# unixpickle/vq-voice-swap

Measured on AMD Instinct MI355X. Metric: audio clips/sec (whole node), unet64 50-step DDPM on 4s@16kHz waveforms, higher is better.
Workload: dtype fp16; 1 GPU; unet64 50-step DDPM (constrain, schedule t**2), 64 clips/GPU x 1 GPU of T=64000; global_batch=64, parallelism=clips sharded over 1 GPU(s), gather to rank 0

## Files before the change

### vq_voice_swap_amd/csrc/common.hpp

```cpp
#pragma once

#include <hip/hip_runtime.h>
#include <stdint.h>

#include <cstdio>
#include <string>

namespace vqvs {

void set_error(const std::string& msg);
#define VQVS_FAIL(code, ...)                        \
  do {                                              \
    char _buf[512];                                 \
    snprintf(_buf, sizeof(_buf), __VA_ARGS__);      \
    ::vqvs::set_error(_buf);                        \
    return (code);                                  \
  } while (0)
#define VQVS_HIP(expr)                                                                       \
  do {                                                                                       \
    hipError_t _e = (expr);                                                                  \
    if (_e != hipSuccess) VQVS_FAIL(-2, "%s failed: %s (%s:%d)", #expr, hipGetErrorString(_e), __FILE__, __LINE__); \
  } while (0)

typedef __bf16 bf16_t;
// ... 55 lines not shown
    f32x2 p = fma2(splat2(0.0000430638f), z, splat2(0.0002765672f));
    p = fma2(p, z, splat2(0.0001520143f));
    p = fma2(p, z, splat2(0.0092705272f));
    p = fma2(p, z, splat2(0.0422820123f));
    p = fma2(p, z, splat2(0.0705230784f));
    p = fma2(p, z, splat2(1.0f));
    p = p * p;
    p = p * p;
    p = p * p;
    p = p * p;
    f32x2 e;
    e[0] = copysignf(1.0f - __builtin_amdgcn_rcpf(p[0]), v[0]);
    e[1] = copysignf(1.0f - __builtin_amdgcn_rcpf(p[1]), v[1]);
    return (v * splat2(0.5f)) * (e + splat2(1.0f));
  } else {
    f32x2 vc;
    vc[0] = __builtin_amdgcn_fmed3f(v[0], -4.0f, 4.0f);
    vc[1] = __builtin_amdgcn_fmed3f(v[1], -4.0f, 4.0f);
    const f32x2 w = vc * vc;
    f32x2 p;
    if constexpr (Q == GELU_POLY6) {
      p = fma2(splat2(2.81608722e-08f), w, splat2(-1.89188380e-06f));
      p = fma2(p, w, splat2(5.41903041e-05f));
      p = fma2(p, w, splat2(-8.78980255e-04f));
      p = fma2(p, w, splat2(9.11294959e-03f));
      p = fma2(p, w, splat2(-6.53883549e-02f));
      p = fma2(p, w, splat2(3.98526915e-01f));
    } else {
      p = fma2(splat2(-1.301278171e-09f), w, splat2(1.041951057e-07f));
      p = fma2(p, w, splat2(-3.657111166e-06f));
      p = fma2(p, w, splat2(7.485478930e-05f));
      p = fma2(p, w, splat2(-1.006488756e-03f));
      p = fma2(p, w, splat2(9.505392772e-03f));
      p = fma2(p, w, splat2(-6.588783436e-02f));
      p = fma2(p, w, splat2(3.986733897e-01f));
    }
    return v * fma2(vc, p, splat2(0.5f));
  }
}
template <typename T> struct GeluQ;
template <> struct GeluQ<float> { static constexpr int q = GELU_EXACT; };
template <> struct GeluQ<bf16_t> { static constexpr int q = GELU_POLY6; };
#ifdef VQVS_F16_GELU6
template <> struct GeluQ<half_t> { static constexpr int q = GELU_POLY6; };
#else
template <> struct GeluQ<half_t> { static constexpr int q = GELU_POLY7; };
#endif

template <typename T>
struct Elem;
template <>
struct Elem<float> {
  static constexpr int BYTES = 4;
  __device__ static __forceinline__ f32x8 load8(const float* p) {
    const f32x4 a = *reinterpret_cast<const f32x4*>(p);
    const f32x4 b = *reinterpret_cast<const f32x4*>(p + 4);
    return f32x8{a[0], a[1], a[2], a[3], b[0], b[1], b[2], b[3]};
  }
  __device__ static __forceinline__ void store8(float* p, f32x8 v) {
    *reinterpret_cast<f32x4*>(p) = f32x4{v[0], v[1], v[2], v[3]};
    *reinterpret_cast<f32x4*>(p + 4) = f32x4{v[4], v[5], v[6], v[7]};
  }
};
template <>
struct Elem<bf16_t> {
  static constexpr int BYTES = 2;
  __device__ static __forceinline__ f32x8 load8(const bf16_t* p) {
    const bf16x8 a = *reinterpret_cast<const bf16x8*>(p);
    return __builtin_convertvector(a, f32x8);
  }
  __device__ static __forceinline__ void store8(bf16_t* p, f32x8 v) {
    *reinterpret_cast<bf16x8*>(p) = __builtin_convertvector(v, bf16x8);
  }
};

template <>
struct Elem<half_t> {
  static constexpr int BYTES = 2;
  __device__ static __forceinline__ f32x8 load8(const half_t* p) {
    const f16x8 a = *reinterpret_cast<const f16x8*>(p);
    return __builtin_convertvector(a, f32x8);
  }
  __device__ static __forceinline__ void store8(half_t* p, f32x8 v) {
    *reinterpret_cast<f16x8*>(p) = __builtin_convertvector(v, f16x8);
  }
};

#define VQVS_BY_PRECISION(precision, CALL) \
  do {                                      \
    if ((precision) == 0) {                 \
      using T = float;                      \
      CALL;                                 \
    } else if ((precision) == 1) {          \
      using T = ::vqvs::bf16_t;             \
      CALL;                                 \
    } else {                                \
      using T = ::vqvs::half_t;             \
      CALL;                                 \
    }                                       \
  } while (0)

__device__ __forceinline__ f32x8 f32x8_zero() { return f32x8{0, 0, 0, 0, 0, 0, 0, 0}; }

__device__ __forceinline__ void split_bf16(f32x8 v, bf16x8& hi, bf16x8& lo) {
  hi = __builtin_convertvector(v, bf16x8);
  const f32x8 r = v - __builtin_convertvector(hi, f32x8);
  lo = __builtin_convertvector(r, bf16x8);
}

}
```

### vq_voice_swap_amd/csrc/kernels.hpp

```cpp
#pragma once

#include "common.hpp"

namespace vqvs {

enum { RESIZE_NONE = 0, RESIZE_AVG2 = 1, RESIZE_UP2 = 2 };

struct SegDesc {
  const void* src;
  const float2* ss;
  long long w_off;
  int Csrc;
  int c0;
  int C;
  int Lsrc;
  int ntaps;
  int dil;
  int resize;
  int ss_stride, ss_c0;
  const void* src2;
  const float4* coef;
  int coef_stride, coef_c0;
};

// ... 48 lines not shown
};
int launch_in_conv(const InConvArgs& a, int B, int precision, hipStream_t st);

struct OutConvArgs {
  const void* in;
  const float2* ss;
  const float* w;
  float bias;
  float* out;
  int C, L;
};
int launch_out_conv(const OutConvArgs& a, int B, int precision, hipStream_t st);

struct GnSrc {
  const float* partials;
  int ntiles, C;
};
struct GnArgs {
  GnSrc src[2];
  int nsrc, Ctot, groups;
  double inv_count;
  const float* gamma;
  const float* beta;
  const float* film;
  int film_stride, film_off;
  float2* ss;
  float2* mr;
  unsigned* status;
  int guard;
};
int launch_gn_prepare(const GnArgs& a, int B, hipStream_t st);

struct TimeEmbedArgs {
  const float* ts;
  const float* freqs;
  const float *w1, *b1;
  const float *w2, *b2;
  const float* class_embed;
  const int64_t* labels;
  int num_labels;
  float* emb;
  float* gemb;
  int E;
};
int launch_time_embed(const TimeEmbedArgs& a, int B, hipStream_t st);
int launch_gelu_rows(const float* in, float* out, int n, hipStream_t st);

struct FilmArgs {
  const float* gemb;
  const float* w;
  const float* bias;
  float* film;
  int E, R;
};
int launch_film(const FilmArgs& a, int B, hipStream_t st);

struct XformArgs {
  const void* in;
  const float2* ss;
  void* out;
  int C, Lin, Lout, avg, ss_stride, ss_c0;
};
int launch_xform(const XformArgs& a, int B, int precision, hipStream_t st);

enum { BW_SAME = 0, BW_FROM_HALF = 1, BW_FROM_DOUBLE = 2 };
struct BwActArgs {
  const void* t;
  const void* xf;
  const float2* ss;
  void* du;
  float* partials;
  int C, L, resize;
  int t_C, t_c0, du_C, du_c0, ss_stride, ss_c0, part_C, part_c0;
};
int launch_bw_act(const BwActArgs& a, int B, int precision, hipStream_t st);

struct GnBwArgs {
  const float* partials;
  int ntiles, C, groups;
  double inv_count;
  const float2* ss;
  const float2* mr;
  float4* coef;
};
int launch_gn_bw(const GnBwArgs& a, int B, hipStream_t st);

struct BwAffineArgs {
  const void* du;
  const void* xf;
  const float4* coef;
  const void* skip;
  int skip_mode;
  const void* extra;
  void* out;
  int C, L;
  int du_C, du_c0, coef_stride, coef_c0, extra_C, extra_c0;
};
int launch_bw_affine(const BwAffineArgs& a, int B, int precision, hipStream_t st);
int launch_bw_add(const void* a, const void* b, void* out, long long n, int precision, hipStream_t st);

struct InConvBwArgs {
  const void* dh;
  const float* w;
  float* out;
  int C, T;
  float out_scale;
// ... 70 lines not shown
```

### vq_voice_swap_amd/csrc/misc_kernels.hip

```cpp
#include <atomic>

#include "kernels.hpp"

namespace vqvs {

namespace {

template <typename T, bool MC>
__global__ __launch_bounds__(256) void in_conv_kernel(const InConvArgs a) {
  __shared__ float red[256 * 8 * 2];
  const int tid = threadIdx.x;
  const int b = blockIdx.y;
  const int t0 = blockIdx.x * STAT_TILE;
  const int opr = a.C >> 3;
  const int rpp = 256 / opr;
  const int oct = tid % opr;
  const int r0 = tid / opr;
  const int c = oct * 8;
  float w0[8], w1[8], w2[8], bs[8];
  const int Cin = MC ? a.Cin : 1;
#pragma unroll
  for (int j = 0; j < 8; ++j) {
    w0[j] = a.w[(c + j) * Cin * 3 + 0];
    w1[j] = a.w[(c + j) * Cin * 3 + 1];
    w2[j] = a.w[(c + j) * Cin * 3 + 2];
    bs[j] = a.bias[c + j];
  }
  const float* xb = a.x + (size_t)b * Cin * a.T;
  f32x8 s1 = f32x8_zero(), s2 = f32x8_zero();
  const bool active = r0 < rpp && oct < opr;
  const float cond_scale = a.condp ? (float)a.cond_len / (float)a.T : 0.f;
  if (active) {
    for (int r = r0; r < STAT_TILE; r += rpp) {
      const int t = t0 + r;
      if (t >= a.T) break;
      const float xm = t > 0 ? xb[t - 1] : 0.f;
      const float x0 = xb[t];
      const float xp = t + 1 < a.T ? xb[t + 1] : 0.f;
      f32x8 v;
#pragma unroll
      for (int j = 0; j < 8; ++j) v[j] = fmaf(w2[j], xp, fmaf(w1[j], x0, fmaf(w0[j], xm, bs[j])));
      if constexpr (MC)
      for (int ci = 1; ci < Cin; ++ci) {
        const float* xc = xb + (size_t)ci * a.T;
        const float ym = t > 0 ? xc[t - 1] : 0.f, y0 = xc[t], yp = t + 1 < a.T ? xc[t + 1] : 0.f;
#pragma unroll
        for (int j = 0; j < 8; ++j) {
          const float* wc = a.w + ((c + j) * Cin + ci) * 3;
          v[j] = fmaf(wc[2], yp, fmaf(wc[1], y0, fmaf(wc[0], ym, v[j])));
        }
      }
      if (a.condp) {
        const int cr = min((int)floorf((float)t * cond_scale), a.cond_len - 1);
        const T* cp = reinterpret_cast<const T*>(a.condp) + ((size_t)b * a.cond_len + cr) * a.C + c;
        v += Elem<T>::load8(cp);
      }
      s1 += v;
      s2 += v * v;
      Elem<T>::store8(reinterpret_cast<T*>(a.out) + ((size_t)b * a.T + t) * a.C + c, v);
    }
  }
  if (active) {
#pragma unroll
    for (int j = 0; j < 8; ++j) {
      red[(r0 * a.C + c + j) * 2 + 0] = s1[j];
      red[(r0 * a.C + c + j) * 2 + 1] = s2[j];
    }
  }
  __syncthreads();
  if (tid < a.C) {
    float t1 = 0.f, t2 = 0.f;
    for (int g = 0; g < rpp; ++g) {
      t1 += red[(g * a.C + tid) * 2 + 0];
      t2 += red[(g * a.C + tid) * 2 + 1];
    }
    float* o = a.stats + (((size_t)b * a.ntiles + blockIdx.x) * a.C + tid) * 2;
    o[0] = t1;
    o[1] = t2;
  }
}

template <typename T>
__global__ __launch_bounds__(256) void out_conv_kernel(const OutConvArgs a) {
  constexpr int GQ = GeluQ<T>::q;
  __shared__ float y[3][STAT_TILE + 2];
  const int tid = threadIdx.x;
  const int b = blockIdx.y;
  const int t0 = blockIdx.x * STAT_TILE;
  const int opr = a.C >> 3;
  const int rpp = 256 / opr;
  const int oct = tid % opr;
  const int r0 = tid / opr;
  const int c = oct * 8;
  f32x8 sc, sh, w0, w1, w2;
  {
    const float2* p = a.ss + (size_t)b * a.C + c;
#pragma unroll
    for (int j = 0; j < 8; ++j) {
      const float2 q = p[j];
      sc[j] = q.x;
      sh[j] = q.y;
      w0[j] = a.w[0 * a.C + c + j];
      w1[j] = a.w[1 * a.C + c + j];
      w2[j] = a.w[2 * a.C + c + j];
    }
  }
  const T* xb = reinterpret_cast<const T*>(a.in) + (size_t)b * a.L * a.C + c;
  for (int r = r0; r < STAT_TILE + 2; r += rpp) {
    const int t = t0 - 1 + r;
    float p0 = 0.f, p1 = 0.f, p2 = 0.f;
    if (t >= 0 && t < a.L) {
      const f32x8 v = Elem<T>::load8(xb + (size_t)t * a.C);
#pragma unroll
      for (int j = 0; j < 8; j += 2) {
        const f32x2 g = gelu2<GQ>(fma2(f32x2{v[j], v[j + 1]}, f32x2{sc[j], sc[j + 1]}, f32x2{sh[j], sh[j + 1]}));
        p0 = fmaf(w0[j + 1], g[1], fmaf(w0[j], g[0], p0));
        p1 = fmaf(w1[j + 1], g[1], fmaf(w1[j], g[0], p1));
        p2 = fmaf(w2[j + 1], g[1], fmaf(w2[j], g[0], p2));
      }
    }
    for (int m = 1; m < opr; m <<= 1) {
      p0 += __shfl_xor(p0, m);
      p1 += __shfl_xor(p1, m);
      p2 += __shfl_xor(p2, m);
    }
    if (oct == 0) {
      y[0][r] = p0;
      y[1][r] = p1;
      y[2][r] = p2;
    }
  }
  __syncthreads();
  const int t = t0 + tid;
  if (t < a.L) a.out[(size_t)b * a.L + t] = a.bias + y[0][tid] + y[1][tid + 1] + y[2][tid + 2];
}

template <typename T>
__global__ __launch_bounds__(256) void out_conv_rows_kernel(const OutConvArgs a) {
  constexpr int GQ = GeluQ<T>::q;
  __shared__ float y[3][STAT_TILE + 2];
  const int tid = threadIdx.x;
  const int b = blockIdx.y;
  const int t0 = blockIdx.x * STAT_TILE;
  const float2* ss = a.ss + (size_t)b * a.C;
  for (int r = tid; r < STAT_TILE + 2; r += 256) {
    const int t = t0 - 1 + r;
    float p0 = 0.f, p1 = 0.f, p2 = 0.f;
    if (t >= 0 && t < a.L) {
      const T* xr = reinterpret_cast<const T*>(a.in) + ((size_t)b * a.L + t) * a.C;
      for (int c = 0; c < a.C; c += 8) {
        const f32x8 v = Elem<T>::load8(xr + c);
#pragma unroll
        for (int j = 0; j < 8; j += 2) {
          const float2 q0 = ss[c + j], q1 = ss[c + j + 1];
          const f32x2 g = gelu2<GQ>(fma2(f32x2{v[j], v[j + 1]}, f32x2{q0.x, q1.x}, f32x2{q0.y, q1.y}));
          p0 = fmaf(a.w[0 * a.C + c + j + 1], g[1], fmaf(a.w[0 * a.C + c + j], g[0], p0));
          p1 = fmaf(a.w[1 * a.C + c + j + 1], g[1], fmaf(a.w[1 * a.C + c + j], g[0], p1));
          p2 = fmaf(a.w[2 * a.C + c + j + 1], g[1], fmaf(a.w[2 * a.C + c + j], g[0], p2));
        }
      }
    }
    y[0][r] = p0;
    y[1][r] = p1;
    y[2][r] = p2;
  }
  __syncthreads();
  const int t = t0 + tid;
  if (t < a.L) a.out[(size_t)b * a.L + t] = a.bias + y[0][tid] + y[1][tid + 1] + y[2][tid + 2];
}

constexpr int GN_SPLIT = 8;

__global__ __launch_bounds__(256) void gn_prepare_kernel(const GnArgs a) {
  __shared__ double part[256 * 2];
  __shared__ double chs[256], chq[256];
  __shared__ double gmean[32], grstd[32];
  const int tid = threadIdx.x;
  const int b = blockIdx.x;
  const int gs = a.Ctot / a.groups;
  const int ng = a.groups / gridDim.y;
  const int c_lo = blockIdx.y * ng * gs;
  const int cw_tot = ng * gs;
  const int C0 = a.src[0].C;
  float pg = 0.f, pb = 0.f, pfa = 0.f, pfb = 0.f;
  if (tid < cw_tot) {
    pg = a.gamma[c_lo + tid];
    pb = a.beta[c_lo + tid];
// ... 81 lines not shown
}

__device__ __forceinline__ float wave_sum(float v) {
#pragma unroll
  for (int m = 32; m >= 1; m >>= 1) v += __shfl_xor(v, m);
  return v;
}

__global__ __launch_bounds__(256) void time_embed_kernel(const TimeEmbedArgs a) {
  __shared__ float e0[1024], e1[1024];
  const int tid = threadIdx.x;
  const int b = blockIdx.x;
  const int E = a.E, half = E >> 1;
  const float t = a.ts[b];
  for (int j = tid; j < half; j += 256) {
    const float arg = t * a.freqs[j];
    e0[j] = cosf(arg);
    e0[half + j] = sinf(arg);
  }
  __syncthreads();
  for (int r = tid; r < E; r += 256) {
    float acc0 = 0.f, acc1 = 0.f, acc2 = 0.f, acc3 = 0.f;
    for (int j = 0; j < E; j += 4) {
      acc0 = fmaf(a.w1[(size_t)(j + 0) * E + r], e0[j + 0], acc0);
      acc1 = fmaf(a.w1[(size_t)(j + 1) * E + r], e0[j + 1], acc1);
      acc2 = fmaf(a.w1[(size_t)(j + 2) * E + r], e0[j + 2], acc2);
      acc3 = fmaf(a.w1[(size_t)(j + 3) * E + r], e0[j + 3], acc3);
    }
    e1[r] = gelu_f((acc0 + acc1) + (acc2 + acc3) + a.b1[r]);
  }
  __syncthreads();
  const float* ce = nullptr;
  if (a.class_embed) {
    long long lab = a.labels[b];
    if (lab < 0) lab = 0;
    if (lab >= a.num_labels) lab = a.num_labels - 1;
    ce = a.class_embed + (size_t)lab * E;
  }
  for (int r = tid; r < E; r += 256) {
    float acc0 = 0.f, acc1 = 0.f, acc2 = 0.f, acc3 = 0.f;
    for (int j = 0; j < E; j += 4) {
      acc0 = fmaf(a.w2[(size_t)(j + 0) * E + r], e1[j + 0], acc0);
      acc1 = fmaf(a.w2[(size_t)(j + 1) * E + r], e1[j + 1], acc1);
      acc2 = fmaf(a.w2[(size_t)(j + 2) * E + r], e1[j + 2], acc2);
      acc3 = fmaf(a.w2[(size_t)(j + 3) * E + r], e1[j + 3], acc3);
    }
    float v = (acc0 + acc1) + (acc2 + acc3) + a.b2[r];
    if (ce) v += ce[r];
    a.emb[(size_t)b * E + r] = v;
    a.gemb[(size_t)b * E + r] = gelu_f(v);
  }
}

__global__ void gelu_rows_kernel(const float* in, float* out, int n) {
  const int i = blockIdx.x * 256 + threadIdx.x;
  if (i < n) out[i] = gelu_f(in[i]);
}

constexpr int FILM_NB = 32;
__global__ __launch_bounds__(256) void film_kernel(const FilmArgs a, int B) {
  extern __shared__ __attribute__((aligned(16))) float fsm[];
  float* const g = fsm;
  float* const red = fsm + a.E * FILM_NB;
  const int lane = threadIdx.x & 63, wv = threadIdx.x >> 6;
  const int r = blockIdx.x * 64 + lane;
  const int E = a.E, b0 = blockIdx.y * FILM_NB;
  const int nb = min(FILM_NB, B - b0);
  for (int i = threadIdx.x; i < E * FILM_NB; i += 256) {
    const int e = i / FILM_NB, bb = i % FILM_NB;
    g[i] = bb < nb ? a.gemb[(size_t)(b0 + bb) * E + e] : 0.f;
  }
  __syncthreads();
  float acc[FILM_NB];
#pragma unroll
  for (int k = 0; k < FILM_NB; ++k) acc[k] = 0.f;
  const int eq = E / 4;
  if (r < a.R) {
    for (int e0 = wv * eq; e0 < (wv + 1) * eq; e0 += 8) {
      float w[8];
#pragma unroll
      for (int u = 0; u < 8; ++u) w[u] = a.w[(size_t)(e0 + u) * a.R + r];
#pragma unroll
      for (int u = 0; u < 8; ++u) {
        const f32x4* gp = reinterpret_cast<const f32x4*>(&g[(e0 + u) * FILM_NB]);
#pragma unroll
        for (int q = 0; q < FILM_NB / 4; ++q) {
          const f32x4 gv = gp[q];
          acc[4 * q + 0] = fmaf(w[u], gv[0], acc[4 * q + 0]);
          acc[4 * q + 1] = fmaf(w[u], gv[1], acc[4 * q + 1]);
          acc[4 * q + 2] = fmaf(w[u], gv[2], acc[4 * q + 2]);
          acc[4 * q + 3] = fmaf(w[u], gv[3], acc[4 * q + 3]);
        }
      }
    }
  }
  if (wv > 0) {
#pragma unroll
    for (int k = 0; k < FILM_NB; ++k) red[((wv - 1) * 64 + lane) * (FILM_NB + 1) + k] = acc[k];
  }
  __syncthreads();
  if (wv == 0 && r < a.R) {
    const float bias = a.bias[r];
#pragma unroll
    for (int k = 0; k < FILM_NB; ++k) {
      float v = acc[k];
#pragma unroll
      for (int w2 = 0; w2 < 3; ++w2) v += red[(w2 * 64 + lane) * (FILM_NB + 1) + k];
      if (k < nb) a.film[(size_t)(b0 + k) * a.R + r] = v + bias;
    }
  }
}

template <typename T>
__global__ __launch_bounds__(256) void xform_kernel(const XformArgs a) {
  constexpr int GQ = GeluQ<T>::q;
  const int b = blockIdx.y;
  const int opr = a.C >> 3;
  const long long item = (long long)blockIdx.x * 256 + threadIdx.x;
  if (item >= (long long)a.Lout * opr) return;
  const int t = (int)(item / opr), c = (int)(item % opr) * 8;
// ... 27 lines not shown

template <typename T>
__global__ __launch_bounds__(256) void nct_to_ntc_kernel(const float* in, T* out, int C, int L) {
  __shared__ float tile[32][33];
  const int b = blockIdx.z, c0 = blockIdx.y * 32, t0 = blockIdx.x * 32;
  const int tx = threadIdx.x & 31, ty = threadIdx.x >> 5;
  for (int i = ty; i < 32; i += 8) {
    const int c = c0 + i, t = t0 + tx;
    tile[i][tx] = (c < C && t < L) ? in[((size_t)b * C + c) * L + t] : 0.f;
  }
  __syncthreads();
  for (int i = ty; i < 32; i += 8) {
    const int t = t0 + i, c = c0 + tx;
    if (t < L && c < C) out[((size_t)b * L + t) * C + c] = (T)tile[tx][i];
  }
}

template <typename T>
__global__ __launch_bounds__(256) void ntc_to_nct_kernel(const T* in, float* out, int C, int L) {
  __shared__ float tile[32][33];
  const int b = blockIdx.z, c0 = blockIdx.y * 32, t0 = blockIdx.x * 32;
  const int tx = threadIdx.x & 31, ty = threadIdx.x >> 5;
  for (int i = ty; i < 32; i += 8) {
    const int t = t0 + i, c = c0 + tx;
    tile[i][tx] = (c < C && t < L) ? (float)in[((size_t)b * L + t) * C + c] : 0.f;
  }
  __syncthreads();
  for (int i = ty; i < 32; i += 8) {
    const int c = c0 + i, t = t0 + tx;
    if (t < L && c < C) out[((size_t)b * C + c) * L + t] = tile[tx][i];
  }
}

template <typename T>
__global__ __launch_bounds__(256) void ntc_stats_kernel(const T* in, float* stats, int C, int L, int ntiles) {
  const int b = blockIdx.y, tile = blockIdx.x;
  const T* p = in + (size_t)b * L * C;
  for (int c = threadIdx.x; c < C; c += 256) {
    float s1 = 0.f, s2 = 0.f;
    const int t1 = min(L, (tile + 1) * STAT_TILE);
    for (int t = tile * STAT_TILE; t < t1; ++t) {
      const float v = (float)p[(size_t)t * C + c];
      s1 += v;
      s2 += v * v;
    }
    float* o = stats + (((size_t)b * ntiles + tile) * C + c) * 2;
    o[0] = s1;
    o[1] = s2;
  }
}

}

int launch_in_conv(const InConvArgs& a, int B, int precision, hipStream_t st) {
  if (a.C % 8 || a.C > 256) VQVS_FAIL(-1, "in_conv: unsupported C=%d", a.C);
  dim3 grid((a.T + STAT_TILE - 1) / STAT_TILE, B);
  if (a.Cin > 1) {
    VQVS_BY_PRECISION(precision, hipLaunchKernelGGL((in_conv_kernel<T, true>), grid, dim3(256), 0, st, a));
  } else {
    VQVS_BY_PRECISION(precision, hipLaunchKernelGGL((in_conv_kernel<T, false>), grid, dim3(256), 0, st, a));
  }
  VQVS_HIP(hipGetLastError());
  return 0;
}

int launch_out_conv(const OutConvArgs& a, int B, int precision, hipStream_t st) {
  const int opr = a.C / 8;
  if (a.C % 8 || opr > 64) VQVS_FAIL(-1, "out_conv: unsupported C=%d", a.C);
  dim3 grid((a.L + STAT_TILE - 1) / STAT_TILE, B);
  if (opr & (opr - 1)) {
    VQVS_BY_PRECISION(precision, hipLaunchKernelGGL(out_conv_rows_kernel<T>, grid, dim3(256), 0, st, a));
  } else {
    VQVS_BY_PRECISION(precision, hipLaunchKernelGGL(out_conv_kernel<T>, grid, dim3(256), 0, st, a));
  }
  VQVS_HIP(hipGetLastError());
  return 0;
}

int launch_gn_prepare(const GnArgs& a, int B, hipStream_t st) {
  if (a.Ctot > 2048 || a.groups > 32 || a.Ctot % a.groups) VQVS_FAIL(-1, "gn: unsupported Ctot=%d groups=%d", a.Ctot, a.groups);
  int split = GN_SPLIT;
  while (split > 1 && (a.groups % split || (a.groups / split) * (a.Ctot / a.groups) > 256)) split >>= 1;
  if ((a.groups / split) * (a.Ctot / a.groups) > 256 && a.Ctot > 256) split = a.groups;
  hipLaunchKernelGGL(gn_prepare_kernel, dim3(B, split), dim3(256), 0, st, a);
  VQVS_HIP(hipGetLastError());
  return 0;
}

int launch_time_embed(const TimeEmbedArgs& a, int B, hipStream_t st) {
  if (a.E > 1024 || a.E % 64) VQVS_FAIL(-1, "time_embed: unsupported E=%d", a.E);
  hipLaunchKernelGGL(time_embed_kernel, dim3(B), dim3(256), 0, st, a);
  VQVS_HIP(hipGetLastError());
  return 0;
}

int launch_gelu_rows(const float* in, float* out, int n, hipStream_t st) {
  hipLaunchKernelGGL(gelu_rows_kernel, dim3((n + 255) / 256), dim3(256), 0, st, in, out, n);
  VQVS_HIP(hipGetLastError());
  return 0;
}

int launch_film(const FilmArgs& a, int B, hipStream_t st) {
  if (a.E > 1024 || a.E < 32 || a.E % 32) VQVS_FAIL(-1, "film: unsupported E=%d", a.E);
  const int lds = (a.E * FILM_NB + 3 * 64 * (FILM_NB + 1)) * 4;
  static std::atomic<bool> attr_done[64];
  int dev = 0;
  if (hipGetDevice(&dev) != hipSuccess || dev < 0 || dev >= 64) dev = 0;
  if (!attr_done[dev].load(std::memory_order_acquire)) {
    VQVS_HIP(hipFuncSetAttribute(reinterpret_cast<const void*>(&film_kernel), hipFuncAttributeMaxDynamicSharedMemorySize, 160 * 1024));
    attr_done[dev].store(true, std::memory_order_release);
  }
  hipLaunchKernelGGL(film_kernel, dim3((a.R + 63) / 64, (B + FILM_NB - 1) / FILM_NB), dim3(256), lds, st, a, B);
  VQVS_HIP(hipGetLastError());
  return 0;
}

int launch_xform(const XformArgs& a, int B, int precision, hipStream_t st) {
  if (a.C % 8) VQVS_FAIL(-1, "xform: unsupported C=%d", a.C);
  const long long items = (long long)a.Lout * (a.C / 8);
  dim3 grid((unsigned)((items + 255) / 256), B);
  VQVS_BY_PRECISION(precision, hipLaunchKernelGGL(xform_kernel<T>, grid, dim3(256), 0, st, a));
  VQVS_HIP(hipGetLastError());
  return 0;
}

int launch_nct_to_ntc(const float* in, void* out, float* stats, int B, int C, int L, int ntiles, int precision, hipStream_t st) {
  dim3 grid((L + 31) / 32, (C + 31) / 32, B);
  VQVS_BY_PRECISION(precision, {
    hipLaunchKernelGGL(nct_to_ntc_kernel<T>, grid, dim3(256), 0, st, in, (T*)out, C, L);
    if (stats) hipLaunchKernelGGL(ntc_stats_kernel<T>, dim3(ntiles, B), dim3(256), 0, st, (const T*)out, stats, C, L, ntiles);
  });
  VQVS_HIP(hipGetLastError());
  return 0;
}

int launch_ntc_to_nct(const void* in, float* out, int B, int C, int L, int in_precision, hipStream_t st) {
  dim3 grid((L + 31) / 32, (C + 31) / 32, B);
  VQVS_BY_PRECISION(in_precision, hipLaunchKernelGGL(ntc_to_nct_kernel<T>, grid, dim3(256), 0, st, (const T*)in, out, C, L));
  VQVS_HIP(hipGetLastError());
  return 0;
}

}
```

### vq_voice_swap_amd/csrc/net.cpp

```cpp
#include "net.hpp"

#include <algorithm>
#include <cmath>
#include <cstring>
#include <functional>
#include <memory>

namespace vqvs {

namespace {

struct Topo {
  std::vector<int> mult;
  int depth = 2;
  std::vector<int> dil;
  int levels() const { return (int)mult.size(); }
};
Topo topo_of(const vqvs_cfg& c) {
  Topo t;
  const bool custom = c.topology_set != 0 && (c.kind == VQVS_KIND_PREDICTOR || c.kind == VQVS_KIND_ENCODER || c.kind == VQVS_KIND_CLASSIFIER);
  if (custom) {
    t.mult.assign(c.channel_mult, c.channel_mult + std::max(0, std::min(c.n_levels, (int)VQVS_MAX_LEVELS)));
    t.depth = c.depth_mult;
    t.dil.assign(c.dilations, c.dilations + std::max(0, std::min(c.n_dilations, 12)));
// ... 1072 lines not shown
      const int Er = 4 * real_base(c);
      const PadMap pm = pad_map(real_base(c));
      for (int i = 0; i < Er / 2; ++i)
        freqs[pm.phys(i)] = (float)(std::exp((double)(float)(-std::log(100.0 / 0.1)) * (double)i / (double)(Er / 2 - 1))) * 100.0f;
    }
    const size_t freq_off = b.blob.add(freqs.data(), freqs.size() * 4);
    const size_t w1 = b.blob_f32_transposed(b.P(px + "time_embed.proj.weight"), E, E), b1 = b.blob_f32(px + "time_embed.proj.bias");
    const size_t w2 = b.blob_f32_transposed(b.P(px + "time_embed_extra.1.weight"), E, E), b2 = b.blob_f32(px + "time_embed_extra.1.bias");
    const size_t ce = c.num_labels > 0 ? b.blob_f32(px + "class_embed.weight") : 0;
    const size_t emb_off = b.alloc_misc((size_t)c.max_batch * E);
    const size_t gemb_off = b.alloc_misc((size_t)c.max_batch * E);
    m->emb_misc_off = emb_off;
    m->emb_E = E;
    const int NL = c.num_labels;
    m->meta.push_back({"time_embed", "", 0, 0, 0});
    m->add_op([=](const RunCtx& r) -> int {
      TimeEmbedArgs a{};
      a.ts = r.ts;
      a.freqs = reinterpret_cast<const float*>(bp->wp(freq_off));
      a.w1 = reinterpret_cast<const float*>(bp->wp(w1));
      a.b1 = reinterpret_cast<const float*>(bp->wp(b1));
      a.w2 = reinterpret_cast<const float*>(bp->wp(w2));
      a.b2 = reinterpret_cast<const float*>(bp->wp(b2));
      a.class_embed = NL > 0 ? reinterpret_cast<const float*>(bp->wp(ce)) : nullptr;
      a.labels = r.labels;
      a.num_labels = NL;
      a.emb = bp->miscp(emb_off);
      a.gemb = bp->miscp(gemb_off);
      a.E = E;
      return launch_time_embed(a, r.B, r.st);
    });
    std::vector<const BlockSpec*> all;
    for (auto& s : d) all.push_back(&s);
    for (auto& s : mdl) all.push_back(&s);
    for (auto& s : u) all.push_back(&s);
    std::vector<int> film_row(all.size());
    int R = 0;
    std::vector<float> Wall, ball;
    for (size_t i = 0; i < all.size(); ++i) {
      film_row[i] = R;
      const float* W = b.P(all[i]->prefix + ".cond_layers.1.weight");
      const float* bb = b.P(all[i]->prefix + ".cond_layers.1.bias");
      const int rows = 2 * all[i]->cout;
      Wall.insert(Wall.end(), W, W + (size_t)rows * E);
      ball.insert(ball.end(), bb, bb + rows);
      R += rows;
    }
    const size_t wall_off = b.blob_f32_transposed(Wall.data(), R, E);
    const size_t ball_off = b.blob.add(ball.data(), ball.size() * 4);
    const size_t film_off = b.alloc_misc((size_t)c.max_batch * R);
    m->meta.push_back({"film", "", 0, 0, 0});
    m->add_op([=](const RunCtx& r) -> int {
      FilmArgs f{bp->miscp(gemb_off), reinterpret_cast<const float*>(bp->wp(wall_off)), reinterpret_cast<const float*>(bp->wp(ball_off)),
                 bp->miscp(film_off), E, R};
      return launch_film(f, r.B, r.st);
    });
    TensorH condp{};
    const bool has_cond = c.cond_channels > 0;
    if (has_cond) {
      const int cond_ls = c.reserved[3] >= LEN_ABS ? c.reserved[3] : (c.reserved[3] == 1 ? LEN_HALF : 8);
      TensorH ct = b.new_tensor(c.cond_channels, cond_ls, false, false);
      const int CC = c.cond_channels;
      m->meta.push_back({"nct_to_ntc", "", 0, 0, 0});
      m->add_op([=](const RunCtx& r) -> int {
        return launch_nct_to_ntc(r.cond, bp->act(ct.off), nullptr, r.B, CC, shiftL(r.Lbase, cond_ls), 0, prec, r.st);
      });
      condp = b.new_tensor(base, cond_ls, false, false);
      PackedConv pk(prec);
      Builder::SegSpec g{ct, 0, CC, 3, 1, RESIZE_NONE, false, 0, 0, 0, 0};
      g.w_off = pk.append(b.P(px + "cond_proj.weight"), base, CC, 3, 0, CC);
      const float* bb = b.P(px + "cond_proj.bias");
      b.add_conv({g}, pk, std::vector<float>(bb, bb + base), base, condp, nullptr, 0);
      b.release(ct);
    }
    TensorH h = b.new_tensor(base, 0, false, true);
    {
      const size_t w = b.blob_f32(px + "in_conv.weight"), bi = b.blob_f32(px + "in_conv.bias");
      const TensorH cp = condp;
      m->meta.push_back({"in_conv", std::to_string(in_ch) + "->" + std::to_string(base), base + (has_cond ? base * lscale(condp.lshift) : 0.0), 4.0 * in_ch, 0});
      m->add_op([=](const RunCtx& r) -> int {
        InConvArgs a{};
        a.x = r.x;
        a.Cin = in_ch;
        a.w = reinterpret_cast<const float*>(bp->wp(w));
        a.bias = reinterpret_cast<const float*>(bp->wp(bi));
        a.condp = has_cond ? bp->act(cp.off) : nullptr;
        a.cond_len = has_cond ? shiftL(r.Lbase, cp.lshift) : 0;
        a.out = bp->act(h.off);
        a.stats = bp->statp(h.stats_off);
        a.C = base;
        a.T = r.Lbase;
        a.ntiles = ntiles_of(r.Lbase);
        return launch_in_conv(a, r.B, prec, r.st);
      });
    }
    if (has_cond) b.release(condp);
    b.tap("in_conv", h);
    std::vector<TensorH> skips{h};
    b.retain(h);
    size_t bi = 0;
    std::vector<Builder::BlockRec> recs(all.size());
    auto recp = [&](size_t i) { return encpred ? &recs[i] : nullptr; };
    for (auto& s : d) {
      TensorH o = b.resblock(s.prefix, s, {h}, true, film_row[bi], R, film_off, recp(bi));
      ++bi;
      b.release(h);
      h = o;
// ... 119 lines not shown
          a.out_scale = r.gscale / grad_scale(prec);
          return launch_in_conv_bw(a, r.B, prec, r.st);
        });
        m->cur_phase = 0;
      }
    }
  } else if (c.kind == VQVS_KIND_CLASSIFIER) {
    const int E = 4 * base, F = classifier_output_mult(c) * base, NL = c.num_labels;
    std::vector<BlockSpec> blocks;
    const int cur = classifier_blocks(base, topo_of(c), blocks);
    b.persist = true;
    std::vector<float> freqs(E / 2);
    for (int i = 0; i < E / 2; ++i)
      freqs[i] = (float)(std::exp((double)(float)(-std::log(100.0 / 0.1)) * (double)i / (double)(E / 2 - 1))) * 100.0f;
    const size_t freq_off = b.blob.add(freqs.data(), freqs.size() * 4);
    const size_t w1 = b.blob_f32_transposed(b.P("stem.time_embed.proj.weight"), E, E), b1 = b.blob_f32("stem.time_embed.proj.bias");
    const size_t w2 = b.blob_f32_transposed(b.P("stem.time_embed_extra.1.weight"), E, E), b2 = b.blob_f32("stem.time_embed_extra.1.bias");
    const size_t emb_off = b.alloc_misc((size_t)c.max_batch * E);
    const size_t gemb_off = b.alloc_misc((size_t)c.max_batch * E);
    m->emb_misc_off = emb_off;
    m->emb_E = E;
    m->meta.push_back({"time_embed", "", 0, 0, 0});
    m->add_op([=](const RunCtx& r) -> int {
      TimeEmbedArgs a{};
      a.ts = r.ts;
      a.freqs = reinterpret_cast<const float*>(bp->wp(freq_off));
      a.w1 = reinterpret_cast<const float*>(bp->wp(w1));
      a.b1 = reinterpret_cast<const float*>(bp->wp(b1));
      a.w2 = reinterpret_cast<const float*>(bp->wp(w2));
      a.b2 = reinterpret_cast<const float*>(bp->wp(b2));
      a.emb = bp->miscp(emb_off);
      a.gemb = bp->miscp(gemb_off);
      a.E = E;
      return launch_time_embed(a, r.B, r.st);
    });
    std::vector<int> film_row(blocks.size());
    int R = 0;
    std::vector<float> Wall, ball;
    for (size_t i = 0; i < blocks.size(); ++i) {
      film_row[i] = R;
      const float* W = b.P(blocks[i].prefix + ".cond_layers.1.weight");
      const float* bb = b.P(blocks[i].prefix + ".cond_layers.1.bias");
      const int rows = 2 * blocks[i].cout;
      Wall.insert(Wall.end(), W, W + (size_t)rows * E);
      ball.insert(ball.end(), bb, bb + rows);
      R += rows;
    }
    const size_t wall_off = b.blob_f32_transposed(Wall.data(), R, E);
    const size_t ball_off = b.blob.add(ball.data(), ball.size() * 4);
    const size_t film_off = b.alloc_misc((size_t)c.max_batch * R);
    m->meta.push_back({"film", "", 0, 0, 0});
    m->add_op([=](const RunCtx& r) -> int {
      FilmArgs f{bp->miscp(gemb_off), reinterpret_cast<const float*>(bp->wp(wall_off)), reinterpret_cast<const float*>(bp->wp(ball_off)),
                 bp->miscp(film_off), E, R};
      return launch_film(f, r.B, r.st);
    });
    TensorH h = b.new_tensor(base, 0, false, true);
    const size_t inw = b.blob_f32("stem.in_conv.weight"), inb = b.blob_f32("stem.in_conv.bias");
    m->meta.push_back({"in_conv", "1->" + std::to_string(base), (double)base, 4.0, 0});
    m->add_op([=](const RunCtx& r) -> int {
      InConvArgs a{};
      a.x = r.x;
      a.w = reinterpret_cast<const float*>(bp->wp(inw));
      a.bias = reinterpret_cast<const float*>(bp->wp(inb));
      a.condp = nullptr;
      a.cond_len = 0;
      a.out = bp->act(h.off);
      a.stats = bp->statp(h.stats_off);
      a.C = base;
      a.T = r.Lbase;
      a.ntiles = ntiles_of(r.Lbase);
      return launch_in_conv(a, r.B, prec, r.st);
    });
    b.tap("stem.in_conv", h);
    std::vector<Builder::BlockRec> recs(blocks.size());
    for (size_t i = 0; i < blocks.size(); ++i) {
      h = b.resblock(blocks[i].prefix, blocks[i], {h}, true, film_row[i], R, film_off, &recs[i]);
      b.tap(blocks[i].prefix, h);
    }
    const size_t ssh = b.alloc_ss(cur), mrh = b.alloc_ss(cur);
    b.add_gn({h}, "stem.out.0.0", false, 0, 0, 0, ssh, true, mrh);
    const int ch = std::min(cur, 64), heads = cur / ch;
    const float* Wqkv = b.P("stem.out.1.qkv_proj.weight");
    const float* bqkv = b.P("stem.out.1.qkv_proj.bias");
    const double sc2 = 1.0 / std::sqrt((double)ch);
    std::vector<float> rvec((size_t)heads * cur), c0(heads);
    for (int hd = 0; hd < heads; ++hd) {
      double cc = 0.0;
      for (int j = 0; j < ch; ++j) cc += (double)bqkv[hd * ch + j] * (double)bqkv[cur + hd * ch + j];
      c0[hd] = (float)(cc * sc2);
      for (int ci = 0; ci < cur; ++ci) {
        double acc = 0.0;
        for (int j = 0; j < ch; ++j) acc += (double)bqkv[hd * ch + j] * (double)Wqkv[(size_t)(cur + hd * ch + j) * cur + ci];
        rvec[(size_t)hd * cur + ci] = (float)(acc * sc2);
      }
    }
    const size_t r_off = b.blob.add(rvec.data(), rvec.size() * 4), c0_off = b.blob.add(c0.data(), c0.size() * 4);
    const size_t wv_off = b.blob.add(Wqkv + (size_t)2 * cur * cur, (size_t)cur * cur * 4);
    const size_t wvT_off = b.blob_f32_transposed(Wqkv + (size_t)2 * cur * cur, cur, cur);
    const size_t wcT_off = b.blob_f32_transposed(b.P("stem.out.1.c_proj.weight"), F, cur);
    const size_t wlT_off = b.blob_f32_transposed(b.P("out.1.weight"), NL, F);
    const size_t bv_off = b.blob.add(bqkv + 2 * cur, (size_t)cur * 4);
    const size_t wc_off = b.blob_f32("stem.out.1.c_proj.weight"), bc_off = b.blob_f32("stem.out.1.c_proj.bias");
    const size_t wl_off = b.blob_f32("out.1.weight"), bl_off = b.blob_f32("out.1.bias");
    b.persist = false;
    TensorH dh = b.new_tensor(cur, h.lshift, false, false);
    const int groups_h = gn_groups(cur);
// ... 276 lines not shown
```

Baseline: 67.98 clips/s.

## Add persistent stream in/out conv kernels, wide time-embed, and shared-timestep FiLM path

Adds grid-stride versions of the single-channel input conv and the output conv. The output conv batches raw fp16 row loads before converting them, and its OPR parameter is a template constant. Time embedding now runs in a 1024-thread kernel that splits each matvec four ways. The FiLM kernel checks at runtime whether every clip in the batch has the same timestep and label; if so, it computes the projection once and broadcasts it to all clips. All of this is on by default and can be switched off with environment variables. The equality check adds a small per-launch scan, and the stream kernels change per-block work and occupancy.

New measurement: 68.26 clips/s, median of 6. Within noise of the previous version (+0.4%).

```diff
diff --git a/vq_voice_swap_amd/csrc/common.hpp b/vq_voice_swap_amd/csrc/common.hpp
--- a/vq_voice_swap_amd/csrc/common.hpp
+++ b/vq_voice_swap_amd/csrc/common.hpp
@@ -131,11 +131,14 @@
 template <>
 struct Elem<float> {
   static constexpr int BYTES = 4;
+  typedef f32x8 raw8;
+  __device__ static __forceinline__ f32x8 cvt8(raw8 a) { return a; }
   __device__ static __forceinline__ f32x8 load8(const float* p) {
     const f32x4 a = *reinterpret_cast<const f32x4*>(p);
     const f32x4 b = *reinterpret_cast<const f32x4*>(p + 4);
     return f32x8{a[0], a[1], a[2], a[3], b[0], b[1], b[2], b[3]};
   }
+  __device__ static __forceinline__ raw8 load8_raw(const float* p) { return load8(p); }
   __device__ static __forceinline__ void store8(float* p, f32x8 v) {
     *reinterpret_cast<f32x4*>(p) = f32x4{v[0], v[1], v[2], v[3]};
     *reinterpret_cast<f32x4*>(p + 4) = f32x4{v[4], v[5], v[6], v[7]};
@@ -144,6 +147,9 @@
 template <>
 struct Elem<bf16_t> {
   static constexpr int BYTES = 2;
+  typedef bf16x8 raw8;
+  __device__ static __forceinline__ raw8 load8_raw(const bf16_t* p) { return *reinterpret_cast<const bf16x8*>(p); }
+  __device__ static __forceinline__ f32x8 cvt8(raw8 a) { return __builtin_convertvector(a, f32x8); }
   __device__ static __forceinline__ f32x8 load8(const bf16_t* p) {
     const bf16x8 a = *reinterpret_cast<const bf16x8*>(p);
     return __builtin_convertvector(a, f32x8);
@@ -156,6 +162,9 @@
 template <>
 struct Elem<half_t> {
   static constexpr int BYTES = 2;
+  typedef f16x8 raw8;
+  __device__ static __forceinline__ raw8 load8_raw(const half_t* p) { return *reinterpret_cast<const f16x8*>(p); }
+  __device__ static __forceinline__ f32x8 cvt8(raw8 a) { return __builtin_convertvector(a, f32x8); }
   __device__ static __forceinline__ f32x8 load8(const half_t* p) {
     const f16x8 a = *reinterpret_cast<const f16x8*>(p);
     return __builtin_convertvector(a, f32x8);
diff --git a/vq_voice_swap_amd/csrc/kernels.hpp b/vq_voice_swap_amd/csrc/kernels.hpp
--- a/vq_voice_swap_amd/csrc/kernels.hpp
+++ b/vq_voice_swap_amd/csrc/kernels.hpp
@@ -124,6 +124,8 @@
   const float* bias;
   float* film;
   int E, R;
+  const float* ts;
+  const int64_t* labels;
 };
 int launch_film(const FilmArgs& a, int B, hipStream_t st);
 
diff --git a/vq_voice_swap_amd/csrc/misc_kernels.hip b/vq_voice_swap_amd/csrc/misc_kernels.hip
--- a/vq_voice_swap_amd/csrc/misc_kernels.hip
+++ b/vq_voice_swap_amd/csrc/misc_kernels.hip
@@ -1,4 +1,5 @@
 #include <atomic>
+#include <cstdlib>
 
 #include "kernels.hpp"
 
@@ -77,6 +78,89 @@
     float* o = a.stats + (((size_t)b * a.ntiles + blockIdx.x) * a.C + tid) * 2;
     o[0] = t1;
     o[1] = t2;
+  }
+}
+
+template <typename T>
+__global__ __launch_bounds__(256) void in_conv_stream_kernel(const InConvArgs a, int nitems) {
+  __shared__ float red[256 * 8 * 2];
+  __shared__ float xs[STAT_TILE + 2];
+  const int tid = threadIdx.x;
+  const int opr = a.C >> 3;
+  const int rpp = 256 / opr;
+  const int oct = tid % opr;
+  const int r0 = tid / opr;
+  const int c = oct * 8;
+  float w0[8], w1[8], w2[8], bs[8];
+  {
+    const f32x4* wp = reinterpret_cast<const f32x4*>(a.w + c * 3);
+    const f32x4* bp = reinterpret_cast<const f32x4*>(a.bias + c);
+    float wf[24];
+#pragma unroll
+    for (int i = 0; i < 6; ++i) {
+      const f32x4 q = wp[i];
+      wf[4 * i + 0] = q[0];
+      wf[4 * i + 1] = q[1];
+      wf[4 * i + 2] = q[2];
+      wf[4 * i + 3] = q[3];
+    }
+    const f32x4 b0 = bp[0], b1 = bp[1];
+#pragma unroll
+    for (int j = 0; j < 8; ++j) {
+      w0[j] = wf[3 * j + 0];
+      w1[j] = wf[3 * j + 1];
+      w2[j] = wf[3 * j + 2];
+      bs[j] = j < 4 ? b0[j & 3] : b1[j & 3];
+    }
+  }
+  const bool active = r0 < rpp;
+  const float cond_scale = a.condp ? (float)a.cond_len / (float)a.T : 0.f;
+  for (int item = blockIdx.x; item < nitems; item += gridDim.x) {
+    const int b = item / a.ntiles, tile = item - b * a.ntiles;
+    const int t0 = tile * STAT_TILE;
+    const float* xb = a.x + (size_t)b * a.T;
+    {
+      const int t = t0 - 1 + tid, t2 = t0 + 255 + (tid & 1);
+      const float xa = xb[min(max(t, 0), a.T - 1)], xc = xb[min(t2, a.T - 1)];
+      xs[tid] = (t >= 0 && t < a.T) ? xa : 0.f;
+      if (tid < 2) xs[256 + tid] = t2 < a.T ? xc : 0.f;
+    }
+    __syncthreads();
+    f32x8 s1 = f32x8_zero(), s2 = f32x8_zero();
+    if (active) {
+      for (int r = r0; r < STAT_TILE; r += rpp) {
+        const int t = t0 + r;
+        if (t >= a.T) break;
+        const float xm = xs[r], x0 = xs[r + 1], xp = xs[r + 2];
+        f32x8 v;
+#pragma unroll
+        for (int j = 0; j < 8; ++j) v[j] = fmaf(w2[j], xp, fmaf(w1[j], x0, fmaf(w0[j], xm, bs[j])));
+        if (a.condp) {
+          const int cr = min((int)floorf((float)t * cond_scale), a.cond_len - 1);
+          const T* cp = reinterpret_cast<const T*>(a.condp) + ((size_t)b * a.cond_len + cr) * a.C + c;
+          v += Elem<T>::load8(cp);
+        }
+        s1 += v;
+        s2 += v * v;
+        Elem<T>::store8(reinterpret_cast<T*>(a.out) + ((size_t)b * a.T + t) * a.C + c, v);
+      }
+#pragma unroll
+      for (int j = 0; j < 8; ++j) {
+        red[(r0 * a.C + c + j) * 2 + 0] = s1[j];
+        red[(r0 * a.C + c + j) * 2 + 1] = s2[j];
+      }
+    }
+    __syncthreads();
+    if (tid < a.C) {
+      float t1 = 0.f, t2 = 0.f;
+      for (int g = 0; g < rpp; ++g) {
+        t1 += red[(g * a.C + tid) * 2 + 0];
+        t2 += red[(g * a.C + tid) * 2 + 1];
+      }
+      float* o = a.stats + (((size_t)b * a.ntiles + tile) * a.C + tid) * 2;
+      o[0] = t1;
+      o[1] = t2;
+    }
   }
 }
 
@@ -133,6 +217,91 @@
   __syncthreads();
   const int t = t0 + tid;
   if (t < a.L) a.out[(size_t)b * a.L + t] = a.bias + y[0][tid] + y[1][tid + 1] + y[2][tid + 2];
+}
+
+template <typename T, int OPR >
+__global__ __launch_bounds__(256) void out_conv_stream_kernel(const OutConvArgs a, int ntiles, int nitems) {
+  constexpr int GQ = GeluQ<T>::q;
+  constexpr int NB = OPR < 8 ? OPR : 8;
+  __shared__ float y[3][STAT_TILE + 2];
+  const int tid = threadIdx.x;
+  constexpr int opr = OPR;
+  constexpr int rpp = 256 / opr;
+  const int oct = tid % opr;
+  const int r0 = tid / opr;
+  const int c = oct * 8;
+  f32x8 w0, w1, w2;
+  {
+    const f32x4* p0 = reinterpret_cast<const f32x4*>(a.w + 0 * a.C + c);
+    const f32x4* p1 = reinterpret_cast<const f32x4*>(a.w + 1 * a.C + c);
+    const f32x4* p2 = reinterpret_cast<const f32x4*>(a.w + 2 * a.C + c);
+    const f32x4 a0 = p0[0], a1 = p0[1], b0 = p1[0], b1 = p1[1], c0 = p2[0], c1 = p2[1];
+    w0 = f32x8{a0[0], a0[1], a0[2], a0[3], a1[0], a1[1], a1[2], a1[3]};
+    w1 = f32x8{b0[0], b0[1], b0[2], b0[3], b1[0], b1[1], b1[2], b1[3]};
+    w2 = f32x8{c0[0], c0[1], c0[2], c0[3], c1[0], c1[1], c1[2], c1[3]};
+  }
+  for (int item = blockIdx.x; item < nitems; item += gridDim.x) {
+    const int b = item / ntiles, tile = item - b * ntiles;
+    const int t0 = tile * STAT_TILE;
+    f32x8 sc, sh;
+    {
+      const f32x4* p = reinterpret_cast<const f32x4*>(a.ss + (size_t)b * a.C + c);
+      const f32x4 q0 = p[0], q1 = p[1], q2 = p[2], q3 = p[3];
+      sc = f32x8{q0[0], q0[2], q1[0], q1[2], q2[0], q2[2], q3[0], q3[2]};
+      sh = f32x8{q0[1], q0[3], q1[1], q1[3], q2[1], q2[3], q3[1], q3[3]};
+    }
+    const T* xb = reinterpret_cast<const T*>(a.in) + (size_t)b * a.L * a.C + c;
+    typedef typename Elem<T>::raw8 raw8;
+    auto row = [&](const raw8 raw, const bool in, const int r) {
+      float p0 = 0.f, p1 = 0.f, p2 = 0.f;
+      const f32x8 v = Elem<T>::cvt8(raw);
+#pragma unroll
+      for (int j = 0; j < 8; j += 2) {
+        const f32x2 g = gelu2<GQ>(fma2(f32x2{v[j], v[j + 1]}, f32x2{sc[j], sc[j + 1]}, f32x2{sh[j], sh[j + 1]}));
+        p0 = fmaf(w0[j + 1], g[1], fmaf(w0[j], g[0], p0));
+        p1 = fmaf(w1[j + 1], g[1], fmaf(w1[j], g[0], p1));
+        p2 = fmaf(w2[j + 1], g[1], fmaf(w2[j], g[0], p2));
+      }
+      p0 = in ? p0 : 0.f;
+      p1 = in ? p1 : 0.f;
+      p2 = in ? p2 : 0.f;
+#pragma unroll
+      for (int m = 1; m < opr; m <<= 1) {
+        p0 += __shfl_xor(p0, m);
+        p1 += __shfl_xor(p1, m);
+        p2 += __shfl_xor(p2, m);
+      }
+      if (oct == 0) {
+        y[0][r] = p0;
+        y[1][r] = p1;
+        y[2][r] = p2;
+      }
+    };
+    const int rh = r0 == 0 ? 0 : STAT_TILE + 1;
+    const int th = t0 - 1 + rh;
+    const bool halo = r0 < 2;
+    const bool hin = halo && th >= 0 && th < a.L;
+    const raw8 vh = Elem<T>::load8_raw(xb + (size_t)(hin ? th : t0) * a.C);
+#pragma unroll 1
+    for (int k0 = 0; k0 < opr; k0 += NB) {
+      raw8 v[NB];
+      bool in[NB];
+#pragma unroll
+      for (int k = 0; k < NB; ++k) {
+        const int t = t0 + r0 + (k0 + k) * rpp;
+        in[k] = t < a.L;
+        v[k] = Elem<T>::load8_raw(xb + (size_t)(in[k] ? t : t0) * a.C);
+      }
+#pragma unroll
+      for (int k = 0; k < NB; ++k)
+        row(v[k], in[k], 1 + r0 + (k0 + k) * rpp);
+    }
+    if (halo) row(vh, hin, rh);
+    __syncthreads();
+    const int t = t0 + tid;
+    if (t < a.L) a.out[(size_t)b * a.L + t] = a.bias + y[0][tid] + y[1][tid + 1] + y[2][tid + 2];
+    __syncthreads();
+  }
 }
 
 template <typename T>
@@ -320,6 +489,54 @@
   }
 }
 
+template <int U>
+__device__ __forceinline__ float te_chain(const float* __restrict__ w, const float* e, int E, int r, int k) {
+  float acc = 0.f;
+  for (int j0 = k; j0 < E; j0 += 4 * U) {
+    float wv[U];
+#pragma unroll
+    for (int u = 0; u < U; ++u) wv[u] = w[(size_t)(j0 + 4 * u) * E + r];
+#pragma unroll
+    for (int u = 0; u < U; ++u) acc = fmaf(wv[u], e[j0 + 4 * u], acc);
+  }
+  return acc;
+}
+
+__global__ __launch_bounds__(1024) void time_embed_wide_kernel(const TimeEmbedArgs a) {
+  __shared__ float e0[1024], e1[1024], part[4][1024];
+  const int tid = threadIdx.x;
+  const int b = blockIdx.x;
+  const int E = a.E, half = E >> 1;
+  const int k = tid >> 8, rl = tid & 255;
+  const float t = a.ts[b];
+  for (int j = tid; j < half; j += 1024) {
+    const float arg = t * a.freqs[j];
+    e0[j] = cosf(arg);
+    e0[half + j] = sinf(arg);
+  }
+  __syncthreads();
+  for (int r = rl; r < E; r += 256) part[k][r] = te_chain<16>(a.w1, e0, E, r, k);
+  __syncthreads();
+  for (int r = tid; r < E; r += 1024)
+    e1[r] = gelu_f((part[0][r] + part[1][r]) + (part[2][r] + part[3][r]) + a.b1[r]);
+  __syncthreads();
+  for (int r = rl; r < E; r += 256) part[k][r] = te_chain<16>(a.w2, e1, E, r, k);
+  __syncthreads();
+  const float* ce = nullptr;
+  if (a.class_embed) {
+    long long lab = a.labels[b];
+    if (lab < 0) lab = 0;
+    if (lab >= a.num_labels) lab = a.num_labels - 1;
+    ce = a.class_embed + (size_t)lab * E;
+  }
+  for (int r = tid; r < E; r += 1024) {
+    float v = (part[0][r] + part[1][r]) + (part[2][r] + part[3][r]) + a.b2[r];
+    if (ce) v += ce[r];
+    a.emb[(size_t)b * E + r] = v;
+    a.gemb[(size_t)b * E + r] = gelu_f(v);
+  }
+}
+
 __global__ void gelu_rows_kernel(const float* in, float* out, int n) {
   const int i = blockIdx.x * 256 + threadIdx.x;
   if (i < n) out[i] = gelu_f(in[i]);
@@ -334,6 +551,46 @@
   const int r = blockIdx.x * 64 + lane;
   const int E = a.E, b0 = blockIdx.y * FILM_NB;
   const int nb = min(FILM_NB, B - b0);
+  if (a.ts) {
+    int diff = 0;
+    const unsigned* tb = reinterpret_cast<const unsigned*>(a.ts);
+    for (int i = threadIdx.x; i < B; i += 256) diff |= (tb[i] != tb[0]) || (a.labels && a.labels[i] != a.labels[0]);
+    int* const differ = reinterpret_cast<int*>(red);
+    if (threadIdx.x == 0) *differ = 0;
+    __syncthreads();
+    if (diff) *differ = 1;
+    __syncthreads();
+    if (*differ == 0) {
+      if (blockIdx.y > 0) return;
+      for (int e = threadIdx.x; e < E; e += 256) g[e] = a.gemb[e];
+      __syncthreads();
+      float acc1 = 0.f;
+      const int eq1 = E / 4;
+      if (r < a.R) {
+        for (int e0 = wv * eq1; e0 < (wv + 1) * eq1; e0 += 8) {
+          float w[8];
+#pragma unroll
+          for (int u = 0; u < 8; ++u) w[u] = a.w[(size_t)(e0 + u) * a.R + r];
+#pragma unroll
+          for (int u = 0; u < 8; ++u) acc1 = fmaf(w[u], g[e0 + u], acc1);
+        }
+      }
+      if (wv > 0) red[(wv - 1) * 64 + lane] = acc1;
+      __syncthreads();
+      if (wv == 0 && r < a.R) {
+        float v = acc1;
+#pragma unroll
+        for (int w2 = 0; w2 < 3; ++w2) v += red[w2 * 64 + lane];
+        red[3 * 64 + lane] = v + a.bias[r];
+      }
+      __syncthreads();
+      if (r < a.R) {
+        const float v = red[3 * 64 + lane];
+        for (int bb = wv; bb < B; bb += 4) a.film[(size_t)bb * a.R + r] = v;
+      }
+      return;
+    }
+  }
   for (int i = threadIdx.x; i < E * FILM_NB; i += 256) {
     const int e = i / FILM_NB, bb = i % FILM_NB;
     g[i] = bb < nb ? a.gemb[(size_t)(b0 + bb) * E + e] : 0.f;
@@ -467,9 +724,43 @@
 
 }
 
+static bool io_stream() {
+  const char* e = getenv("VQVS_IO_STREAM");
+  return e ? atoi(e) != 0 : true;
+}
+static bool film_once() {
+  const char* e = getenv("VQVS_FILM_ONCE");
+  return e ? atoi(e) != 0 : true;
+}
+static int io_num_cus() {
+  static std::atomic<int> n[64];
+  int dev = 0;
+  if (hipGetDevice(&dev) != hipSuccess || dev < 0 || dev >= 64) dev = 0;
+  int v = n[dev].load(std::memory_order_relaxed);
+  if (v == 0) {
+    hipDeviceProp_t p;
+    v = (hipGetDeviceProperties(&p, dev) == hipSuccess && p.multiProcessorCount > 0) ? p.multiProcessorCount : 256;
+    n[dev].store(v, std::memory_order_relaxed);
+  }
+  return v;
+}
+static int io_grid(int nitems) {
+  const char* e = getenv("VQVS_IO_GRID");
+  const int per_cu = e ? atoi(e) : 0;
+  if (per_cu == 0) return nitems;
+  const int n = per_cu < 0 ? -per_cu : io_num_cus() * per_cu;
+  return n < nitems ? n : nitems;
+}
+
 int launch_in_conv(const InConvArgs& a, int B, int precision, hipStream_t st) {
   if (a.C % 8 || a.C > 256) VQVS_FAIL(-1, "in_conv: unsupported C=%d", a.C);
   dim3 grid((a.T + STAT_TILE - 1) / STAT_TILE, B);
+  if (a.Cin <= 1 && io_stream() && a.ntiles == (int)grid.x) {
+    const int nitems = a.ntiles * B;
+    VQVS_BY_PRECISION(precision, hipLaunchKernelGGL(in_conv_stream_kernel<T>, dim3(io_grid(nitems)), dim3(256), 0, st, a, nitems));
+    VQVS_HIP(hipGetLastError());
+    return 0;
+  }
   if (a.Cin > 1) {
     VQVS_BY_PRECISION(precision, hipLaunchKernelGGL((in_conv_kernel<T, true>), grid, dim3(256), 0, st, a));
   } else {
@@ -483,6 +774,19 @@
   const int opr = a.C / 8;
   if (a.C % 8 || opr > 64) VQVS_FAIL(-1, "out_conv: unsupported C=%d", a.C);
   dim3 grid((a.L + STAT_TILE - 1) / STAT_TILE, B);
+  if (!(opr & (opr - 1)) && opr >= 4 && io_stream()) {
+    const int ntiles = (int)grid.x, nitems = ntiles * B;
+    const dim3 g1(io_grid(nitems));
+    switch (opr) {
+      case 4: VQVS_BY_PRECISION(precision, hipLaunchKernelGGL((out_conv_stream_kernel<T, 4>), g1, dim3(256), 0, st, a, ntiles, nitems)); break;
+      case 8: VQVS_BY_PRECISION(precision, hipLaunchKernelGGL((out_conv_stream_kernel<T, 8>), g1, dim3(256), 0, st, a, ntiles, nitems)); break;
+      case 16: VQVS_BY_PRECISION(precision, hipLaunchKernelGGL((out_conv_stream_kernel<T, 16>), g1, dim3(256), 0, st, a, ntiles, nitems)); break;
+      case 32: VQVS_BY_PRECISION(precision, hipLaunchKernelGGL((out_conv_stream_kernel<T, 32>), g1, dim3(256), 0, st, a, ntiles, nitems)); break;
+      default: VQVS_BY_PRECISION(precision, hipLaunchKernelGGL((out_conv_stream_kernel<T, 64>), g1, dim3(256), 0, st, a, ntiles, nitems)); break;
+    }
+    VQVS_HIP(hipGetLastError());
+    return 0;
+  }
   if (opr & (opr - 1)) {
     VQVS_BY_PRECISION(precision, hipLaunchKernelGGL(out_conv_rows_kernel<T>, grid, dim3(256), 0, st, a));
   } else {
@@ -504,7 +808,11 @@
 
 int launch_time_embed(const TimeEmbedArgs& a, int B, hipStream_t st) {
   if (a.E > 1024 || a.E % 64) VQVS_FAIL(-1, "time_embed: unsupported E=%d", a.E);
-  hipLaunchKernelGGL(time_embed_kernel, dim3(B), dim3(256), 0, st, a);
+  if (film_once()) {
+    hipLaunchKernelGGL(time_embed_wide_kernel, dim3(B), dim3(1024), 0, st, a);
+  } else {
+    hipLaunchKernelGGL(time_embed_kernel, dim3(B), dim3(256), 0, st, a);
+  }
   VQVS_HIP(hipGetLastError());
   return 0;
 }
@@ -525,7 +833,9 @@
     VQVS_HIP(hipFuncSetAttribute(reinterpret_cast<const void*>(&film_kernel), hipFuncAttributeMaxDynamicSharedMemorySize, 160 * 1024));
     attr_done[dev].store(true, std::memory_order_release);
   }
-  hipLaunchKernelGGL(film_kernel, dim3((a.R + 63) / 64, (B + FILM_NB - 1) / FILM_NB), dim3(256), lds, st, a, B);
+  FilmArgs f = a;
+  if (!film_once()) f.ts = nullptr;
+  hipLaunchKernelGGL(film_kernel, dim3((a.R + 63) / 64, (B + FILM_NB - 1) / FILM_NB), dim3(256), lds, st, f, B);
   VQVS_HIP(hipGetLastError());
   return 0;
 }
diff --git a/vq_voice_swap_amd/csrc/net.cpp b/vq_voice_swap_amd/csrc/net.cpp
--- a/vq_voice_swap_amd/csrc/net.cpp
+++ b/vq_voice_swap_amd/csrc/net.cpp
@@ -1148,7 +1148,7 @@
     m->meta.push_back({"film", "", 0, 0, 0});
     m->add_op([=](const RunCtx& r) -> int {
       FilmArgs f{bp->miscp(gemb_off), reinterpret_cast<const float*>(bp->wp(wall_off)), reinterpret_cast<const float*>(bp->wp(ball_off)),
-                 bp->miscp(film_off), E, R};
+                 bp->miscp(film_off), E, R, r.ts, NL > 0 ? r.labels : nullptr};
       return launch_film(f, r.B, r.st);
     });
     TensorH condp{};
@@ -1374,7 +1374,7 @@
     m->meta.push_back({"film", "", 0, 0, 0});
     m->add_op([=](const RunCtx& r) -> int {
       FilmArgs f{bp->miscp(gemb_off), reinterpret_cast<const float*>(bp->wp(wall_off)), reinterpret_cast<const float*>(bp->wp(ball_off)),
-                 bp->miscp(film_off), E, R};
+                 bp->miscp(film_off), E, R, r.ts, nullptr};
       return launch_film(f, r.B, r.st);
     });
     TensorH h = b.new_tensor(base, 0, false, true);
```
